# KatherLab/STAMP

Hardware: AMD Instinct MI355X
Metric: tiles/sec encoded (224x224, ViT-L/14) (higher is better)
Workload: dtype f16

## Files before the change

stamp_amd/csrc/gemm_4w16.h:

```cpp
#pragma once
#include <type_traits>
#include "gemm_kernel.h"

namespace amds {

__device__ __forceinline__ f32x4 agpr_read(const f32x4& a) {
    f32x4 v;
    asm("v_accvgpr_read_b32 %0, %1" : "=v"(v[0]) : "a"(a[0]));
    asm("v_accvgpr_read_b32 %0, %1" : "=v"(v[1]) : "a"(a[1]));
    asm("v_accvgpr_read_b32 %0, %1" : "=v"(v[2]) : "a"(a[2]));
    asm("v_accvgpr_read_b32 %0, %1" : "=v"(v[3]) : "a"(a[3]));
    return v;
}

template <typename T, int EPI, int P3 = 6, int P0 = 6, bool SPREAD = true, int PRL = 0, int PRS = 0, bool TN = false>
__global__ void __launch_bounds__(256) __attribute__((amdgpu_waves_per_eu(1, 1)))
gemm_4w16_kernel(const T* __restrict__ A, long lda, const T* __restrict__ W, long ldw, int M, int N, int K,
                 EpiArgs ep, int tiles_m, int tiles_n) {
    typedef typename Act<T>::vec8 vec8;
    typedef typename Act<T>::vec4 vec4;
    constexpr int BM = 256, BN = 256, BK = 64, NT = 256;
    constexpr int ROWB = BK * 2;
    constexpr int A_BYTES = BM * ROWB, STAGE = (BM + BN) * ROWB;
    constexpr int FI = 8, FJ = 8;
    constexpr int GROUP_M = 8;

    extern __shared__ __attribute__((aligned(16))) char smem[];

    const int tid = threadIdx.x;
    const int lane = tid & 63;
    const int wave = __builtin_amdgcn_readfirstlane(tid >> 6);
    const int wm = wave >> 1, wn = wave & 1;
    const int l15 = lane & 15, kb = lane >> 4;
    const int l31 = lane & 31, hi = lane >> 5;

    int tm, tn;
    {
        const int nwg = gridDim.x, bid = blockIdx.x;
        const int xcd = bid & 7, q = nwg >> 3, r = nwg & 7;
        const int t = (xcd < r ? xcd * (q + 1) : r * (q + 1) + (xcd - r) * q) + (bid >> 3);
        const int group = GROUP_M * tiles_n;
        const int g = t / group, first_m = g * GROUP_M;
        const int gm = min(tiles_m - first_m, GROUP_M);
        const int rr = t - g * group;
        tm = first_m + rr % gm;
        tn = rr / gm;
    }
    const int m0 = tm * BM, n0 = tn * BN;
    if (ep.nbatch > 1) {
        const long by = blockIdx.y;
        A += by * ep.bsA;
        W += by * ep.bsW;
        constexpr bool F32O = (EPI == AMDS_EPI_RESIDUAL || EPI == AMDS_EPI_BIAS_F32 || EPI == AMDS_EPI_BIAS_GELU_F32 || EPI == AMDS_EPI_BIAS_RELU_F32);
        if (F32O) ep.out = reinterpret_cast<float*>(ep.out) + by * ep.bsOut;
        else ep.out = reinterpret_cast<T*>(ep.out) + by * ep.bsOut;
    }

    const int rows_a = min(BM, M - m0);
    const long tn_valid = TN ? (ep.ktot > 0 ? min((long)K, ep.ktot - (long)blockIdx.y * K) : (long)K) : 0;
    const __amdgpu_buffer_rsrc_t rsrc_a = TN ? __builtin_amdgcn_make_buffer_rsrc(const_cast<T*>(A + m0), 0, tn_valid > 0 ? (int)(((tn_valid - 1) * lda + BM) * 2) : 0, 0x00020000)
                                             : __builtin_amdgcn_make_buffer_rsrc(const_cast<T*>(A + (long)m0 * lda), 0, (int)((((long)rows_a - 1) * lda + K) * 2), 0x00020000);
    const __amdgpu_buffer_rsrc_t rsrc_w = TN ? __builtin_amdgcn_make_buffer_rsrc(const_cast<T*>(W + n0), 0, tn_valid > 0 ? (int)(((tn_valid - 1) * ldw + BN) * 2) : 0, 0x00020000)
                                             : __builtin_amdgcn_make_buffer_rsrc(const_cast<T*>(W + (long)n0 * ldw), 0, (int)(((long)(BN - 1) * ldw + K) * 2), 0x00020000);
    int voff[16];
#pragma unroll
    for (int it = 0; it < 16; ++it) {
        if constexpr (TN) {
            const int c = (it & 7) * NT + tid, row = c >> 5, pos = c & 31, g = (row & 3) | ((row >> 1) & 4);
            voff[it] = (int)(((long)row * (it < 8 ? lda : ldw) + (pos ^ (g << 1)) * 8) * 2);
        } else {
            const int c = (it & 7) * NT + tid, row = c >> 3, cp = c & 7, sc = cp ^ ((row >> 1) & 7);
            voff[it] = (int)(((long)row * (it < 8 ? lda : ldw) + sc * 8) * 2);
        }
    }
    auto issue_pieces = [&](int kt, int lo, int hi_) {
        char* st = smem + (kt & 1) * STAGE;
        const int koff = TN ? kt * BK * (int)lda * 2 : kt * BK * 2;
        const int koff_w = TN ? kt * BK * (int)ldw * 2 : koff;
#pragma unroll
        for (int it = 0; it < 16; ++it)
            if (it >= lo && it < hi_) {
                if (it < 8) {
                    __builtin_amdgcn_raw_ptr_buffer_load_lds(rsrc_a, (lptr_t)(st + ((it & 7) * NT + wave * 64) * 16), 16, voff[it], koff, 0, 0);
                } else {
                    __builtin_amdgcn_raw_ptr_buffer_load_lds(rsrc_w, (lptr_t)(st + A_BYTES + ((it & 7) * NT + wave * 64) * 16), 16, voff[it], koff_w,
                                                             0, 0);
                }
            }
    };

    const int swz = (l15 >> 1) & 7;
    const int a_off = (wm * 128 + l15) * ROWB;
    const int w_off = A_BYTES + (wn * 128 + l15) * ROWB;

    const bool lnf = ep.rowstat != nullptr;
    const bool bias_in_acc = ep.bias != nullptr && ep.acc_scale == 1.0f && !lnf;
    f32x4 acc[FI][FJ];
    {
        f32x4 b0[FJ];
#pragma unroll
        for (int j = 0; j < FJ; ++j) b0[j] = f32x4{0.f, 0.f, 0.f, 0.f};
        if (bias_in_acc) {
#pragma unroll
            for (int j = 0; j < FJ; ++j) b0[j] = *reinterpret_cast<const f32x4*>(ep.bias + n0 + wn * 128 + j * 16 + 4 * kb);
        }
        __builtin_amdgcn_sched_barrier(0);
        issue_pieces(0, 0, 16);
        if constexpr (P3 < 0) {
            if (K / BK > 1) issue_pieces(1, 0, 16);
        }
        __builtin_amdgcn_sched_barrier(0);
#pragma unroll
        for (int i = 0; i < FI; ++i)
#pragma unroll
            for (int j = 0; j < FJ; ++j) acc[i][j] = b0[j];
    }
#pragma unroll
    for (int i = 0; i < FI; ++i) {
        if (i == FI - 1)
            asm volatile("s_nop 7" : "+a"(acc[i][0]), "+a"(acc[i][1]), "+a"(acc[i][2]), "+a"(acc[i][3]), "+a"(acc[i][4]), "+a"(acc[i][5]),
                         "+a"(acc[i][6]), "+a"(acc[i][7]));
        else
            asm volatile("" : "+a"(acc[i][0]), "+a"(acc[i][1]), "+a"(acc[i][2]), "+a"(acc[i][3]), "+a"(acc[i][4]), "+a"(acc[i][5]),
                         "+a"(acc[i][6]), "+a"(acc[i][7]));
    }
    __builtin_amdgcn_sched_barrier(0);

    vec8 af[2][FI], wf[2][FJ];
    const int tn_g = (l15 >> 2) | ((kb & 1) << 2);
    const int tn_row = (kb * 8 + (l15 >> 2)) * 512 + (l15 & 1) * 8 + ((l15 >> 1) & 1) * 16;
    auto load_frags = [&](int kt, int ks, int s, int lo, int hi_) {
        const char* sb = smem + (kt & 1) * STAGE;
        if constexpr (TN) {
            const unsigned base = (unsigned)(size_t)(sb + tn_row + ks * 32 * 512);
#pragma unroll
            for (int q = 0; q < 16; ++q)
                if (q >= lo && q < hi_) {
                    const int qq = q & 7;
                    const unsigned pq = base + (q < 8 ? 0 : A_BYTES) + ((q < 8 ? wm : wn) * 16 + 2 * (qq ^ tn_g)) * 16;
                    u32x2 a0, a1;
                    asm volatile("ds_read_b64_tr_b16 %0, %1" : "=v"(a0) : "v"(pq) : "memory");
                    asm volatile("ds_read_b64_tr_b16 %0, %1 offset:2048" : "=v"(a1) : "v"(pq) : "memory");
                    const vec8 f = __builtin_bit_cast(vec8, u32x4{a0[0], a0[1], a1[0], a1[1]});
                    if (q < 8) af[s][qq] = f; else wf[s][qq] = f;
                }
        } else {
            const int co = ((ks * 4 + kb) ^ swz) << 4;
#pragma unroll
            for (int q = 0; q < 16; ++q)
                if (q >= lo && q < hi_) {
                    if (q < 8) af[s][q] = *reinterpret_cast<const vec8*>(sb + a_off + q * 16 * ROWB + co);
                    else wf[s][q - 8] = *reinterpret_cast<const vec8*>(sb + w_off + (q - 8) * 16 * ROWB + co);
                }
        }
    };
    auto unit = [&](int s, int ih, auto nr_c, int rkt, int rks, int rs, int rlo, auto nc_c, int ckt, int clo) {
        constexpr int NR = decltype(nr_c)::value, NC = decltype(nc_c)::value;
        constexpr int R_SPAN = SPREAD ? (NR >= 16 ? 16 : 32) : (NR > 0 ? NR : 1), C_LO = SPREAD ? (NR >= 16 ? 16 : 0) : NR,
                      C_SPAN = SPREAD ? 32 - C_LO : (NC > 0 ? NC : 1);
#pragma unroll
        for (int m = 0; m < 32; ++m) {
            Act<T>::mfma16_agpr(wf[s][m & 7], af[s][ih * 4 + (m >> 3)], acc[ih * 4 + (m >> 3)][m & 7]);
            if (NR > 0 && m < R_SPAN) {
                const int r0 = m * NR / R_SPAN, r1 = (m + 1) * NR / R_SPAN;
                if (r1 > r0) load_frags(rkt, rks, rs, rlo + r0, rlo + r1);
            }
            if (NC > 0 && m >= C_LO && m < C_LO + C_SPAN) {
                const int c0 = (m - C_LO) * NC / C_SPAN, c1 = (m - C_LO + 1) * NC / C_SPAN;
// ... 199 lines not shown
                    *reinterpret_cast<vec4*>(smem + row * 256 + ((chunk ^ (row & 15)) << 4) + half) = Act<T>::from_f32x4(o);
                }
        }
        __syncthreads();
        const int l15r = lane & 15, rsub = lane >> 4;
#pragma unroll 4
        for (int it = 0; it < 16; ++it) {
            const int row = wave * 64 + it * 4 + rsub;
            const u32x4 v = *reinterpret_cast<const u32x4*>(smem + row * 256 + l15r * 16);
            const int chunk = l15r ^ (row & 15);
            if (m0 + row < M)
                *reinterpret_cast<u32x4*>(reinterpret_cast<T*>(ep.out) + (long)(m0 + row) * ep.ldo + n0 / 2 + chunk * 8) = v;
        }
        return;
    }
    if constexpr (EPI == AMDS_EPI_RESIDUAL) {
        if (rmw_fast) {
            const int rows_o = min(BM, M - m0);
            rsrc_o = __builtin_amdgcn_make_buffer_rsrc(reinterpret_cast<float*>(ep.out) + (long)m0 * ep.ldo + n0, 0,
                                                       (int)((((long)rows_o - 1) * ep.ldo + BN) * 4), 0x00020000);
#pragma unroll
            for (int h = 0; h < 2; ++h)
#pragma unroll
                for (int u = 0; u < 8; ++u)
                    offu[h][u] = (wave * 64 + 2 * u + hi) * ldo4 + (((l31 >> 4) ^ h) << 9) + (((l31 & 15) ^ (2 * u + hi)) << 4);
            const __amdgpu_buffer_rsrc_t rsrc_h = __builtin_amdgcn_make_buffer_rsrc(
                ep.xh ? reinterpret_cast<T*>(ep.xh) + (long)m0 * ep.ldo + n0 : reinterpret_cast<T*>(ep.out), 0,
                ep.xh ? (int)((((long)rows_o - 1) * ep.ldo + BN) * 2) : 0, 0x00020000);
            const __amdgpu_buffer_rsrc_t rsrc_l = __builtin_amdgcn_make_buffer_rsrc(
                ep.xl ? reinterpret_cast<T*>(ep.xl) + (long)m0 * ep.ldo + n0 : reinterpret_cast<T*>(ep.out), 0,
                ep.xl ? (int)((((long)rows_o - 1) * ep.ldo + BN) * 2) : 0, 0x00020000);
            const int np_part = N / 128;
            auto run = [&](auto has_scale_c, auto lnp_c, auto pl_c) {
                constexpr bool HS = decltype(has_scale_c)::value, LNP = decltype(lnp_c)::value, PL = decltype(pl_c)::value;
                auto load_prev = [&](int pass, int b8) {
                    if constexpr (PL) {
                        int rowoff = b8 * 16 * ldo4 + pass * 256;
                        asm volatile("" : "+s"(rowoff));
#pragma unroll
                        for (int u = 0; u < 8; ++u) {
                            const int o = (offu[b8 & 1][u] + rowoff) >> 1;
                            const u32x2 ph = __builtin_bit_cast(u32x2, __builtin_amdgcn_raw_buffer_load_b64(rsrc_h, o, 0, 0));
                            const u32x2 pl = __builtin_bit_cast(u32x2, __builtin_amdgcn_raw_buffer_load_b64(rsrc_l, o, 0, 0));
                            old[b8][u] = __builtin_bit_cast(f32x4, u32x4{ph[0], ph[1], pl[0], pl[1]});
                        }
                    } else {
                        load_old(pass, b8);
                    }
                };
                f32x4 sc[4];
                auto load_scale = [&](int pass) {
                    if constexpr (HS) {
#pragma unroll
                        for (int jj = 0; jj < 4; ++jj)
                            sc[jj] = *reinterpret_cast<const f32x4*>(ep.scale + n0 + wn * 128 + (pass * 4 + jj) * 16 + 4 * kb);
                    }
                };
                load_scale(0);
#pragma unroll
                for (int b8 = 0; b8 < 4; ++b8) load_prev(0, b8);
#pragma unroll
                for (int pass = 0; pass < 2; ++pass) {
#pragma unroll
                    for (int i = 0; i < FI; ++i) {
                        const int row = wm * 128 + i * 16 + l15;
#pragma unroll
                        for (int jj = 0; jj < 4; ++jj) {
                            f32x4 v = agpr_read(acc[i][pass * 4 + jj]);
                            if constexpr (HS) v *= sc[jj];
                            const int chunk = wn * 16 + jj * 4 + kb;
                            *reinterpret_cast<f32x4*>(smem + row * 512 + ((chunk ^ (row & 31)) << 4)) = v;
                        }
                        __builtin_amdgcn_sched_barrier(0);
                    }
                    asm volatile("s_waitcnt lgkmcnt(0)" ::: "memory");
                    __builtin_amdgcn_sched_barrier(0);
                    __builtin_amdgcn_s_barrier();
                    __builtin_amdgcn_sched_barrier(0);
                    if (pass == 0) load_scale(1);
#pragma unroll
                    for (int b8 = 0; b8 < 4; ++b8) {
                        f32x4 v[8];
#pragma unroll
                        for (int u = 0; u < 8; ++u) {
                            const int row = wave * 64 + (b8 * 8 + u) * 2 + hi;
                            v[u] = *reinterpret_cast<const f32x4*>(smem + row * 512 + l31 * 16);
                        }
                        int rowoff = b8 * 16 * ldo4 + pass * 256;
                        asm volatile("" : "+s"(rowoff));
#pragma unroll
                        for (int u = 0; u < 8; ++u) {
                            if constexpr (PL) {
                                const u32x4 o = __builtin_bit_cast(u32x4, old[b8][u]);
                                const vec4 h4 = __builtin_bit_cast(vec4, u32x2{o[0], o[1]}), l4 = __builtin_bit_cast(vec4, u32x2{o[2], o[3]});
                                f32x4 old4;
                                if constexpr (std::is_same<T, f16>::value) {
                                    old4 = f32x4{mix_add_hh<0, 0>(o[0], o[2]), mix_add_hh<1, 1>(o[0], o[2]), mix_add_hh<0, 0>(o[1], o[3]), mix_add_hh<1, 1>(o[1], o[3])};
                                } else {
                                    old4 = __builtin_convertvector(h4, f32x4) + __builtin_convertvector(l4, f32x4);
                                }
                                v[u] += old4;
                            } else {
                                v[u] += old[b8][u];
                                __builtin_amdgcn_raw_buffer_store_b128(__builtin_bit_cast(u32x4, v[u]), rsrc_o, offu[b8 & 1][u] + rowoff, 0, 0);
                            }
                        }
                        if constexpr (LNP) {
                            f32x2 ss[8];
#pragma unroll
                            for (int u = 0; u < 8; ++u) {
                                const vec4 c = Act<T>::from_f32x4(v[u]);
                                __builtin_amdgcn_raw_buffer_store_b64(__builtin_bit_cast(u32x2, c), rsrc_h, (offu[b8 & 1][u] + rowoff) >> 1, 0, 0);
                                if constexpr (PL) {
                                    f32x4 rest;
                                    if constexpr (std::is_same<T, f16>::value) {
                                        const u32x2 cu = __builtin_bit_cast(u32x2, c);
                                        rest = f32x4{mix_sub_fh<0>(v[u][0], cu[0]), mix_sub_fh<1>(v[u][1], cu[0]), mix_sub_fh<0>(v[u][2], cu[1]), mix_sub_fh<1>(v[u][3], cu[1])};
                                    } else {
                                        rest = v[u] - __builtin_convertvector(c, f32x4);
                                    }
                                    const vec4 cl = Act<T>::from_f32x4(rest);
                                    __builtin_amdgcn_raw_buffer_store_b64(__builtin_bit_cast(u32x2, cl), rsrc_l, (offu[b8 & 1][u] + rowoff) >> 1, 0, 0);
                                }
                                ss[u] = f32x2{(v[u][0] + v[u][1]) + (v[u][2] + v[u][3]),
                                              fmaf(v[u][0], v[u][0], v[u][1] * v[u][1]) + fmaf(v[u][2], v[u][2], v[u][3] * v[u][3])};
                            }
                            const f32x2 tot = half_wave_sum8(ss, l31);
                            const int urow = ((l31 >> 4) & 1) * 4 + ((l31 >> 3) & 1) * 2 + ((l31 >> 2) & 1);
                            const int prow = m0 + wave * 64 + b8 * 16 + 2 * urow + hi;
                            if ((l31 & 3) == 0 && prow < M)
                                *reinterpret_cast<f32x2*>(ep.rowpart + ((long)prow * np_part + tn * 2 + pass) * 2) = tot;
                        }
                        if (pass == 0) load_prev(1, b8);
                        __builtin_amdgcn_sched_barrier(0);
                    }
                    if (pass == 0) {
                        asm volatile("s_waitcnt lgkmcnt(0)" ::: "memory");
                        __builtin_amdgcn_sched_barrier(0);
                        __builtin_amdgcn_s_barrier();
                        __builtin_amdgcn_sched_barrier(0);
                    }
                }
            };
            if (ep.xl) {
                if (ep.scale) run(std::true_type{}, std::true_type{}, std::true_type{}); else run(std::false_type{}, std::true_type{}, std::true_type{});
            } else if (ep.xh) {
                if (ep.scale) run(std::true_type{}, std::true_type{}, std::false_type{}); else run(std::false_type{}, std::true_type{}, std::false_type{});
            } else {
                if (ep.scale) run(std::true_type{}, std::false_type{}, std::false_type{}); else run(std::false_type{}, std::false_type{}, std::false_type{});
            }
            return;
        }
    }
    constexpr int NPASS = F16OUT ? 1 : 2;
    constexpr int JP = FJ / NPASS;
#pragma unroll
    for (int pass = 0; pass < NPASS; ++pass) {
        if (pass) __syncthreads();
        EpiArgs epv = ep;
        if (bias_in_acc || lnf) epv.bias = nullptr;
        EpiCols<JP> cols;
        epi_cols_load<EPI>(epv, cols, [&](int jj) { return n0 + wn * 128 + (pass * JP + jj) * 16 + 4 * kb; });
        auto values = [&](auto fast_c) {
            constexpr bool FAST = decltype(fast_c)::value;
#pragma unroll
            for (int i = 0; i < FI; ++i) {
                const int row = wm * 128 + i * 16 + l15;
#pragma unroll
                for (int jj = 0; jj < JP; jj += 2) {
                    const int j = pass * JP + jj;
                    f32x4 v0 = agpr_read(acc[i][j]), v1 = agpr_read(acc[i][j + 1]);
                    epi_value_pair<EPI, FAST, true>(epv, cols.bias[jj], cols.scale[jj], cols.bias[jj + 1], cols.scale[jj + 1], v0, v1);
                    if constexpr (F16OUT) {
                        const vec4 o0 = Act<T>::from_f32x4(v0), o1 = Act<T>::from_f32x4(v1);
                        const int chunk = wn * 16 + j * 2 + (kb >> 1);
                        const int half = ((kb & 1) ^ ((l15 >> 3) & 1)) * 8;
                        *reinterpret_cast<vec4*>(smem + row * 512 + ((chunk ^ (row & 31)) << 4) + half) = o0;
                        *reinterpret_cast<vec4*>(smem + row * 512 + (((chunk + 2) ^ (row & 31)) << 4) + half) = o1;
                    } else {
                        const int chunk = wn * 16 + jj * 4 + kb;
                        *reinterpret_cast<f32x4*>(smem + row * 512 + ((chunk ^ (row & 31)) << 4)) = v0;
                        *reinterpret_cast<f32x4*>(smem + row * 512 + (((chunk + 4) ^ (row & 31)) << 4)) = v1;
                    }
                }
            }
        };
        auto values_ln = [&]() {
            if constexpr (LNC && F16OUT) {
#pragma unroll
                for (int i = 0; i < FI; ++i) {
                    const int row = wm * 128 + i * 16 + l15;
#pragma unroll
                    for (int j = 0; j < FJ; j += 2) {
                        f32x4 v0 = agpr_read(acc[i][j]), v1 = agpr_read(acc[i][j + 1]);
                        v0 = v0 * rs[i][0] + (cs[j] * rs[i][1] + cb[j]);
                        v1 = v1 * rs[i][0] + (cs[j + 1] * rs[i][1] + cb[j + 1]);
                        epi_value_pair<EPI, true, true>(epv, cb[j], cb[j], cb[j + 1], cb[j + 1], v0, v1);
                        const vec4 o0 = Act<T>::from_f32x4(v0), o1 = Act<T>::from_f32x4(v1);
                        const int chunk = wn * 16 + j * 2 + (kb >> 1);
                        const int half = ((kb & 1) ^ ((l15 >> 3) & 1)) * 8;
                        *reinterpret_cast<vec4*>(smem + row * 512 + ((chunk ^ (row & 31)) << 4) + half) = o0;
                        *reinterpret_cast<vec4*>(smem + row * 512 + (((chunk + 2) ^ (row & 31)) << 4) + half) = o1;
                    }
                }
            }
        };
        if (LNC && F16OUT && lnf) values_ln();
        else if (F16OUT && (bias_in_acc || (ep.bias == nullptr && ep.acc_scale == 1.0f))) values(std::true_type{}); else values(std::false_type{});
        __syncthreads();
#pragma unroll 1
        for (int b8 = 0; b8 < 4; ++b8) {
            if constexpr (F16OUT) {
                u32x4 v[8];
#pragma unroll
                for (int u = 0; u < 8; ++u) {
                    const int row = wave * 64 + (b8 * 8 + u) * 2 + hi;
                    v[u] = *reinterpret_cast<const u32x4*>(smem + row * 512 + l31 * 16);
                    if ((u >> 2) & 1) v[u] = u32x4{v[u][2], v[u][3], v[u][0], v[u][1]};
                }
#pragma unroll
                for (int u = 0; u < 8; ++u) {
                    const int row = wave * 64 + (b8 * 8 + u) * 2 + hi;
                    const int chunk = l31 ^ (row & 31);
                    if (m0 + row < M)
                        *reinterpret_cast<u32x4*>(reinterpret_cast<T*>(ep.out) + (long)(m0 + row) * ep.ldo + n0 + chunk * 8) = v[u];
                }
            } else {
                f32x4 v[8], o[8];
#pragma unroll
                for (int u = 0; u < 8; ++u) {
                    const int row = wave * 64 + (b8 * 8 + u) * 2 + hi;
                    const int chunk = l31 ^ (row & 31);
                    const int n = n0 + (chunk >> 4) * 128 + pass * 64 + (chunk & 15) * 4;
                    v[u] = *reinterpret_cast<const f32x4*>(smem + row * 512 + l31 * 16);
                    if constexpr (EPI == AMDS_EPI_RESIDUAL)
                        o[u] = *reinterpret_cast<const f32x4*>(reinterpret_cast<const float*>(ep.out) +
                                                               (long)min(m0 + row, M - 1) * ep.ldo + n);
                }
#pragma unroll
                for (int u = 0; u < 8; ++u) {
                    const int row = wave * 64 + (b8 * 8 + u) * 2 + hi;
                    const int chunk = l31 ^ (row & 31);
                    const int n = n0 + (chunk >> 4) * 128 + pass * 64 + (chunk & 15) * 4;
                    if constexpr (EPI == AMDS_EPI_RESIDUAL) v[u] += o[u];
                    if (m0 + row < M)
                        *reinterpret_cast<f32x4*>(reinterpret_cast<float*>(ep.out) + (long)(m0 + row) * ep.ldo + n) = v[u];
                }
            }
        }
    }
}

template <typename T, int EPI, bool SPREAD = true, int P3 = 6, int P0 = 6, int PRL = 0, int PRS = 0, bool TN = false>
static int launch_gemm_4w16(const void* A, long lda, const void* W, long ldw, int M, int N, int K, const EpiArgs& ep,
                            hipStream_t st) {
    if constexpr (!epi_is_staged<EPI>() && EPI != AMDS_EPI_SWIGLU) {
        return launch_gemm_4w64<T, EPI>(A, lda, W, ldw, M, N, K, ep, st);
    } else {
        constexpr int LDS = 2 * (256 + 256) * 128;
        constexpr auto kern = gemm_4w16_kernel<T, EPI, P3, P0, SPREAD, PRL, PRS, TN>;
        EpiArgs epp = ep;
        if constexpr (PRL + PRS > 0) {
            static char* scratch = nullptr;
            static size_t scratch_bytes = 0;
            const size_t need = (size_t)cdiv(M, 256) * (N / 256) * (K / 64) * 4096 * (PRL > PRS ? PRL : PRS);
            if (need > scratch_bytes) {
                if (scratch) AMDS_HIP(hipFree(scratch));
                AMDS_HIP(hipMalloc(reinterpret_cast<void**>(&scratch), need));
                scratch_bytes = need;
            }
            epp.pos = reinterpret_cast<const float*>(scratch);
        }
        AMDS_HIP(lds_opt_in<kern>(LDS));
        const int tiles_m = cdiv(M, 256), tiles_n = N / 256;
        hipLaunchKernelGGL(kern, dim3(tiles_m * tiles_n, ep.nbatch), dim3(256), LDS, st, reinterpret_cast<const T*>(A), lda,
                           reinterpret_cast<const T*>(W), ldw, M, N, K, epp, tiles_m, tiles_n);
        AMDS_LAUNCH_CHECK("gemm_4w16_kernel");
        return AMDS_OK;
    }
}

}
```

stamp_amd/csrc/gemm_kernel.h:

```cpp
#pragma once
#include <type_traits>
#include "launch.h"

namespace amds {

struct EpiArgs {
    void* out;
    long ldo;
    const float* bias;
    const float* scale;
    const float* pos;
    int np, T, P;
    float acc_scale;
    long bsA = 0, bsW = 0, bsOut = 0;
    int nbatch = 1;
    void* xh = nullptr;
    void* xl = nullptr;
    float* rowpart = nullptr;
    const float* rowstat = nullptr;
    const float* colsum = nullptr;
    long ktot = 0;
};

template <int EPI>
constexpr bool epi_is_staged() {
    return EPI == AMDS_EPI_BIAS || EPI == AMDS_EPI_BIAS_GELU || EPI == AMDS_EPI_BIAS_RELU || EPI == AMDS_EPI_RESIDUAL ||
           EPI == AMDS_EPI_BIAS_F32 || EPI == AMDS_EPI_BIAS_GELU_F32 || EPI == AMDS_EPI_BIAS_RELU_F32;
}

template <int G>
struct EpiCols {
    f32x4 bias[G], scale[G];
};
template <int EPI, int G, typename F>
__device__ __forceinline__ void epi_cols_load(const EpiArgs& ep, EpiCols<G>& c, F col_of) {
    if (ep.bias) {
#pragma unroll
        for (int q = 0; q < G; ++q) c.bias[q] = *reinterpret_cast<const f32x4*>(ep.bias + col_of(q));
    }
    if constexpr (EPI == AMDS_EPI_RESIDUAL) {
        if (ep.scale) {
#pragma unroll
            for (int q = 0; q < G; ++q) c.scale[q] = *reinterpret_cast<const f32x4*>(ep.scale + col_of(q));
        }
    }
}

template <int EPI>
__device__ __forceinline__ f32x4 epi_value(const EpiArgs& ep, const f32x4& bias, const f32x4& scale, f32x4 v) {
    if (ep.acc_scale != 1.0f) v *= ep.acc_scale;
    if (ep.bias) v += bias;
    if constexpr (EPI == AMDS_EPI_BIAS_GELU) {
        const f32x2 a = gelu_erf_poly2(f32x2{v[0], v[1]}), b = gelu_erf_poly2(f32x2{v[2], v[3]});
        v = f32x4{a[0], a[1], b[0], b[1]};
    }
    if constexpr (EPI == AMDS_EPI_BIAS_GELU_F32) {
#pragma unroll
        for (int e = 0; e < 4; ++e) v[e] = gelu_erf(v[e]);
    }
    if constexpr (EPI == AMDS_EPI_BIAS_RELU || EPI == AMDS_EPI_BIAS_RELU_F32) {
#pragma unroll
        for (int e = 0; e < 4; ++e) v[e] = fmaxf(v[e], 0.f);
    }
    if constexpr (EPI == AMDS_EPI_RESIDUAL) {
        if (ep.scale) v *= scale;
    }
    return v;
}

template <int EPI, bool FAST, bool NOBIAS = false>
__device__ __forceinline__ void epi_value_pair(const EpiArgs& ep, const f32x4& b0, const f32x4& s0, const f32x4& b1, const f32x4& s1,
                                               f32x4& v0, f32x4& v1) {
    if constexpr (FAST && EPI == AMDS_EPI_BIAS_GELU) {
        if constexpr (!NOBIAS) {
            v0 += b0;
            v1 += b1;
        }
        f32x2 q[4] = {f32x2{v0[0], v0[1]}, f32x2{v0[2], v0[3]}, f32x2{v1[0], v1[1]}, f32x2{v1[2], v1[3]}};
        gelu_erf_poly2_n<4>(q);
        v0 = f32x4{q[0][0], q[0][1], q[1][0], q[1][1]};
        v1 = f32x4{q[2][0], q[2][1], q[3][0], q[3][1]};
    } else if constexpr (FAST && (EPI == AMDS_EPI_BIAS || EPI == AMDS_EPI_BIAS_RELU)) {
        if constexpr (!NOBIAS) {
            v0 += b0;
            v1 += b1;
        }
        if constexpr (EPI == AMDS_EPI_BIAS_RELU) {
#pragma unroll
            for (int e = 0; e < 4; ++e) { v0[e] = fmaxf(v0[e], 0.f); v1[e] = fmaxf(v1[e], 0.f); }
        }
    } else {
        v0 = epi_value<EPI>(ep, b0, s0, v0);
        v1 = epi_value<EPI>(ep, b1, s1, v1);
    }
}

template <int EPI, typename T>
__device__ __forceinline__ void epilogue4(const EpiArgs& ep, int m, int n, float v0, float v1, float v2,
                                          float v3) {
    typedef typename Act<T>::vec4 vec4;
    if (ep.acc_scale != 1.0f) { v0 *= ep.acc_scale; v1 *= ep.acc_scale; v2 *= ep.acc_scale; v3 *= ep.acc_scale; }
    if constexpr (EPI != AMDS_EPI_SWIGLU) {
        if (ep.bias) {
            const f32x4 b = *reinterpret_cast<const f32x4*>(ep.bias + n);
            v0 += b[0]; v1 += b[1]; v2 += b[2]; v3 += b[3];
        }
    }
    if constexpr (EPI == AMDS_EPI_BIAS_GELU) {
        v0 = gelu_erf_fast(v0); v1 = gelu_erf_fast(v1); v2 = gelu_erf_fast(v2); v3 = gelu_erf_fast(v3);
    }
    if constexpr (EPI == AMDS_EPI_BIAS_GELU_F32) {
        v0 = gelu_erf(v0); v1 = gelu_erf(v1); v2 = gelu_erf(v2); v3 = gelu_erf(v3);
    }
    if constexpr (EPI == AMDS_EPI_BIAS_RELU || EPI == AMDS_EPI_BIAS_RELU_F32) {
        v0 = fmaxf(v0, 0.f); v1 = fmaxf(v1, 0.f); v2 = fmaxf(v2, 0.f); v3 = fmaxf(v3, 0.f);
    }
    if constexpr (EPI == AMDS_EPI_BIAS || EPI == AMDS_EPI_BIAS_GELU || EPI == AMDS_EPI_BIAS_RELU) {
        vec4 o;
        o[0] = Act<T>::from_f32(v0); o[1] = Act<T>::from_f32(v1);
        o[2] = Act<T>::from_f32(v2); o[3] = Act<T>::from_f32(v3);
        *reinterpret_cast<vec4*>(reinterpret_cast<T*>(ep.out) + (long)m * ep.ldo + n) = o;
    } else if constexpr (EPI == AMDS_EPI_BIAS_F32 || EPI == AMDS_EPI_BIAS_GELU_F32 ||
                         EPI == AMDS_EPI_BIAS_RELU_F32) {
        f32x4 o = {v0, v1, v2, v3};
        *reinterpret_cast<f32x4*>(reinterpret_cast<float*>(ep.out) + (long)m * ep.ldo + n) = o;
    } else if constexpr (EPI == AMDS_EPI_RESIDUAL) {
        if (ep.scale) {
            const f32x4 s = *reinterpret_cast<const f32x4*>(ep.scale + n);
            v0 *= s[0]; v1 *= s[1]; v2 *= s[2]; v3 *= s[3];
        }
        f32x4* p = reinterpret_cast<f32x4*>(reinterpret_cast<float*>(ep.out) + (long)m * ep.ldo + n);
        f32x4 x = *p;
        x[0] += v0; x[1] += v1; x[2] += v2; x[3] += v3;
        *p = x;
    } else if constexpr (EPI == AMDS_EPI_PATCH) {
        const int b = m / ep.np, pi = m - b * ep.np;
        const f32x4 pe = *reinterpret_cast<const f32x4*>(ep.pos + (long)pi * ep.ldo + n);
        f32x4 o = {v0 + pe[0], v1 + pe[1], v2 + pe[2], v3 + pe[3]};
        *reinterpret_cast<f32x4*>(reinterpret_cast<float*>(ep.out) +
                                  ((long)b * ep.T + ep.P + pi) * ep.ldo + n) = o;
    }
}

template <typename T, int BM, int BN, int WM, int WN, int EPI>
__global__ void __launch_bounds__(64 * WM * WN) __attribute__((amdgpu_waves_per_eu(2, 2)))
gemm_tn_kernel(const T* __restrict__ A, long lda, const T* __restrict__ W, long ldw, int M, int N, int K,
               EpiArgs ep, int tiles_m, int tiles_n) {
    typedef typename Act<T>::vec8 vec8;
    typedef typename Act<T>::vec4 vec4;
    constexpr int NT = 64 * WM * WN;
    constexpr int BK = 64;
    constexpr int WTM = BM / WM, WTN = BN / WN;
    constexpr int FM = WTM / 32, FN = WTN / 32;
// ... 59 lines not shown
    const int w_row_off = A_BYTES + (wn * WTN + l31) * 128;

    f32x16 acc[FM][FN];
#pragma unroll
    for (int i = 0; i < FM; ++i)
#pragma unroll
        for (int j = 0; j < FN; ++j)
#pragma unroll
            for (int r = 0; r < 16; ++r) acc[i][j][r] = 0.f;

    const int nk = K / BK;
    stage_load(0, 0);
    vec8 af[2][FM], wf[2][FN];
    auto load_frags = [&](const char* sb, int ks, int set) {
        const int coff = ((ks * 2 + hi) ^ swz) << 4;
#pragma unroll
        for (int i = 0; i < FM; ++i)
            af[set][i] = *reinterpret_cast<const vec8*>(sb + a_row_off + i * 32 * 128 + coff);
#pragma unroll
        for (int j = 0; j < FN; ++j)
            wf[set][j] = *reinterpret_cast<const vec8*>(sb + w_row_off + j * 32 * 128 + coff);
    };
    for (int kt = 0; kt < nk; ++kt) {
        asm volatile("s_waitcnt vmcnt(0)" ::: "memory");
        __syncthreads();
        if (kt + 1 < nk) stage_load((kt + 1) & 1, kt + 1);
        const char* sb = smem + (kt & 1) * STAGE;
        load_frags(sb, 0, 0);
#pragma unroll
        for (int ks = 0; ks < 4; ++ks) {
            if (ks + 1 < 4) load_frags(sb, ks + 1, (ks + 1) & 1);
#pragma unroll
            for (int i = 0; i < FM; ++i)
#pragma unroll
                for (int j = 0; j < FN; ++j)
                    acc[i][j] = Act<T>::mfma32(wf[ks & 1][j], af[ks & 1][i], acc[i][j]);
            if (ks + 1 < 4) {
#pragma unroll
                for (int r = 0; r < PAIRS; ++r) {
                    __builtin_amdgcn_sched_group_barrier(0x008, 1, 0);
                    __builtin_amdgcn_sched_group_barrier(0x100, 1, 0);
                }
                if constexpr (FM * FN > PAIRS) __builtin_amdgcn_sched_group_barrier(0x008, FM * FN - PAIRS, 0);
                if constexpr (FM + FN > PAIRS) __builtin_amdgcn_sched_group_barrier(0x100, FM + FN - PAIRS, 0);
            }
        }
    }

    if constexpr (epi_is_staged<EPI>()) {
        constexpr bool F16OUT = (EPI == AMDS_EPI_BIAS || EPI == AMDS_EPI_BIAS_GELU || EPI == AMDS_EPI_BIAS_RELU);
        constexpr int CPR = BN * (F16OUT ? 2 : 4) / 16, PITCH = (CPR | 1) * 16;
        EpiCols<FN * 4> cols;
        epi_cols_load<EPI>(ep, cols, [&](int q) { return n0 + wn * WTN + (q >> 2) * 32 + 8 * (q & 3) + 4 * hi; });
        __syncthreads();
#pragma unroll
        for (int i = 0; i < FM; ++i) {
            const int row = wm * WTM + i * 32 + l31;
#pragma unroll
            for (int j = 0; j < FN; ++j)
#pragma unroll
                for (int g = 0; g < 4; ++g) {
                    const int nl = wn * WTN + j * 32 + 8 * g + 4 * hi;
                    f32x4 v = {acc[i][j][4 * g], acc[i][j][4 * g + 1], acc[i][j][4 * g + 2], acc[i][j][4 * g + 3]};
                    v = epi_value<EPI>(ep, cols.bias[j * 4 + g], cols.scale[j * 4 + g], v);
                    if constexpr (F16OUT) {
                        vec4 o;
#pragma unroll
                        for (int e = 0; e < 4; ++e) o[e] = Act<T>::from_f32(v[e]);
                        *reinterpret_cast<vec4*>(smem + row * PITCH + nl * 2) = o;
                    } else {
                        *reinterpret_cast<f32x4*>(smem + row * PITCH + nl * 4) = v;
                    }
                }
        }
        __syncthreads();
        for (int idx = tid; idx < BM * CPR; idx += NT) {
            const int row = idx / CPR, c = idx - row * CPR;
            if (m0 + row < M) {
                if constexpr (F16OUT) {
                    const u32x4 v = *reinterpret_cast<const u32x4*>(smem + row * PITCH + c * 16);
                    *reinterpret_cast<u32x4*>(reinterpret_cast<T*>(ep.out) + (long)(m0 + row) * ep.ldo + n0 + c * 8) = v;
                } else {
                    f32x4 v = *reinterpret_cast<const f32x4*>(smem + row * PITCH + c * 16);
                    f32x4* p = reinterpret_cast<f32x4*>(reinterpret_cast<float*>(ep.out) + (long)(m0 + row) * ep.ldo + n0 + c * 4);
                    if constexpr (EPI == AMDS_EPI_RESIDUAL) v += *p;
                    *p = v;
                }
            }
        }
    } else {
#pragma unroll
    for (int i = 0; i < FM; ++i) {
        const int m = m0 + wm * WTM + i * 32 + l31;
        if (m < M) {
            if constexpr (EPI == AMDS_EPI_SWIGLU) {
#pragma unroll
                for (int j = 0; j < FN; j += 2) {
                    const int hbase = (n0 + wn * WTN + j * 32) / 2;
#pragma unroll
                    for (int g = 0; g < 4; ++g) {
                        const int hcol = hbase + 8 * g + 4 * hi;
                        float gte[4], val[4];
                        const f32x4 bg = *reinterpret_cast<const f32x4*>(
                            ep.bias + n0 + wn * WTN + j * 32 + 8 * g + 4 * hi);
                        const f32x4 bv = *reinterpret_cast<const f32x4*>(
                            ep.bias + n0 + wn * WTN + (j + 1) * 32 + 8 * g + 4 * hi);
                        vec4 o;
#pragma unroll
                        for (int e = 0; e < 4; ++e) {
                            gte[e] = acc[i][j][4 * g + e] * ep.acc_scale + bg[e];
                            val[e] = acc[i][j + 1][4 * g + e] * ep.acc_scale + bv[e];
                            o[e] = Act<T>::from_f32(silu(gte[e]) * val[e]);
                        }
                        *reinterpret_cast<vec4*>(reinterpret_cast<T*>(ep.out) + (long)m * ep.ldo + hcol) = o;
                    }
                }
            } else {
#pragma unroll
                for (int j = 0; j < FN; ++j)
#pragma unroll
                    for (int g = 0; g < 4; ++g) {
                        const int n = n0 + wn * WTN + j * 32 + 8 * g + 4 * hi;
                        epilogue4<EPI, T>(ep, m, n, acc[i][j][4 * g + 0], acc[i][j][4 * g + 1],
                                          acc[i][j][4 * g + 2], acc[i][j][4 * g + 3]);
                    }
            }
        }
    }
    }
}

template <typename T, int BM, int BN, int WM, int WN, int EPI>
static int launch_gemm_cfg(const void* A, long lda, const void* W, long ldw, int M, int N, int K,
                           const EpiArgs& ep, hipStream_t st) {
    constexpr int STAGE = (BM + BN) * 64 * 2;
    constexpr int EPI_LDS = BM * ((BN * 4 / 16) | 1) * 16;
    constexpr int LDS = 2 * STAGE > EPI_LDS ? 2 * STAGE : EPI_LDS;
    constexpr auto kern = gemm_tn_kernel<T, BM, BN, WM, WN, EPI>;
    AMDS_HIP(lds_opt_in<kern>(LDS));
    const int tiles_m = cdiv(M, BM), tiles_n = N / BN;
    hipLaunchKernelGGL(kern, dim3(tiles_m * tiles_n), dim3(64 * WM * WN), LDS, st,
                       reinterpret_cast<const T*>(A), lda, reinterpret_cast<const T*>(W), ldw, M, N, K, ep,
                       tiles_m, tiles_n);
    AMDS_LAUNCH_CHECK("gemm_tn_kernel");
    return AMDS_OK;
}

template <typename T, int EPI>
static int launch_gemm_8p64(const void* A, long lda, const void* W, long ldw, int M, int N, int K, const EpiArgs& ep,
                            hipStream_t st);
template <typename T, int EPI>
static int launch_gemm_4w64(const void* A, long lda, const void* W, long ldw, int M, int N, int K, const EpiArgs& ep,
                            hipStream_t st);
template <typename T, int EPI, bool SPREAD, int P3, int P0, int PRL, int PRS, bool TN>
static int launch_gemm_4w16(const void* A, long lda, const void* W, long ldw, int M, int N, int K, const EpiArgs& ep,
                            hipStream_t st);

template <typename T, int EPI>
static int launch_gemm(int cfg, const void* A, long lda, const void* W, long ldw, int M, int N, int K,
                       const EpiArgs& ep, hipStream_t st) {
    if (cfg == 10 && N % 256 == 0 && ep.nbatch == 1) return launch_gemm_4w64<T, EPI>(A, lda, W, ldw, M, N, K, ep, st);
    if (cfg == 10) cfg = 8;
    if (cfg == 12 && N % 256 == 0) return launch_gemm_4w16<T, EPI, true, 6, 6, 0, 0, false>(A, lda, W, ldw, M, N, K, ep, st);
    if (cfg == 13 && N % 256 == 0) return launch_gemm_4w16<T, EPI, true, -2, 0, 0, 0, false>(A, lda, W, ldw, M, N, K, ep, st);
#ifdef AMDS_GEMM_PROBE
    if constexpr (EPI == AMDS_EPI_BIAS || EPI == AMDS_EPI_BIAS_GELU || EPI == AMDS_EPI_RESIDUAL) {
        if (cfg == 21 && N % 256 == 0) return launch_gemm_4w16<T, EPI, true, 6, 6, 0, 2, false>(A, lda, W, ldw, M, N, K, ep, st);
        if (cfg == 22 && N % 256 == 0) return launch_gemm_4w16<T, EPI, true, 6, 6, 1, 1, false>(A, lda, W, ldw, M, N, K, ep, st);
        if (cfg == 23 && N % 256 == 0) return launch_gemm_4w16<T, EPI, true, 6, 6, 4, 4, false>(A, lda, W, ldw, M, N, K, ep, st);
    }
#endif
    if constexpr (EPI == AMDS_EPI_BIAS_F32) {
        if (cfg == 15 && N % 256 == 0 && M % 256 == 0) return launch_gemm_4w16<T, EPI, true, 6, 6, 0, 0, true>(A, lda, W, ldw, M, N, K, ep, st);
    }
    if (cfg == 15) { set_error("amds_gemm: kernel 15 (token-major operands) takes the BIAS_F32 epilogue and M, N multiples of 256"); return AMDS_ERR_INVALID; }
    if (cfg == 12 || cfg == 13) cfg = 8;

    if (cfg == 8 && N % 256 == 0) return launch_gemm_8p64<T, EPI>(A, lda, W, ldw, M, N, K, ep, st);
    if (cfg == 8) cfg = 0;
    if (cfg == 0 && N % 128 != 0) cfg = 1;
    switch (cfg) {
        case 0: return launch_gemm_cfg<T, 128, 128, 2, 2, EPI>(A, lda, W, ldw, M, N, K, ep, st);
        case 1:
            if constexpr (EPI == AMDS_EPI_SWIGLU || EPI == AMDS_EPI_PATCH) {
                set_error("amds_gemm: the 128x96 tile has no SWIGLU / PATCH epilogue");
                return AMDS_ERR_INVALID;
            } else {
                if (N % 96 != 0) { set_error("amds_gemm: kernel 1 needs N %% 96 == 0 (N=%d)", N); return AMDS_ERR_INVALID; }
                return launch_gemm_cfg<T, 128, 96, 4, 1, EPI>(A, lda, W, ldw, M, N, K, ep, st);
            }
    }
    set_error("amds_gemm: unknown tile config %d", cfg);
    return AMDS_ERR_INVALID;
}

template <typename T>
int gemm_dispatch(int cfg, int epi, const void* A, long lda, const void* W, long ldw, int M, int N, int K,
                  const EpiArgs& ep, hipStream_t st);

#define AMDS_GEMM_DISPATCH_IMPL(T)                                                                        \
    template <>                                                                                           \
    int gemm_dispatch<T>(int cfg, int epi, const void* A, long lda, const void* W, long ldw, int M, int N, \
                         int K, const EpiArgs& ep, hipStream_t st) {                                      \
        switch (epi) {                                                                                    \
            case AMDS_EPI_BIAS: return launch_gemm<T, AMDS_EPI_BIAS>(cfg, A, lda, W, ldw, M, N, K, ep, st); \
            case AMDS_EPI_BIAS_GELU: return launch_gemm<T, AMDS_EPI_BIAS_GELU>(cfg, A, lda, W, ldw, M, N, K, ep, st); \
            case AMDS_EPI_BIAS_RELU: return launch_gemm<T, AMDS_EPI_BIAS_RELU>(cfg, A, lda, W, ldw, M, N, K, ep, st); \
            case AMDS_EPI_RESIDUAL: return launch_gemm<T, AMDS_EPI_RESIDUAL>(cfg, A, lda, W, ldw, M, N, K, ep, st); \
            case AMDS_EPI_BIAS_F32: return launch_gemm<T, AMDS_EPI_BIAS_F32>(cfg, A, lda, W, ldw, M, N, K, ep, st); \
            case AMDS_EPI_SWIGLU: return launch_gemm<T, AMDS_EPI_SWIGLU>(cfg, A, lda, W, ldw, M, N, K, ep, st); \
            case AMDS_EPI_PATCH: return launch_gemm<T, AMDS_EPI_PATCH>(cfg, A, lda, W, ldw, M, N, K, ep, st); \
            case AMDS_EPI_BIAS_GELU_F32: return launch_gemm<T, AMDS_EPI_BIAS_GELU_F32>(cfg, A, lda, W, ldw, M, N, K, ep, st); \
            case AMDS_EPI_BIAS_RELU_F32: return launch_gemm<T, AMDS_EPI_BIAS_RELU_F32>(cfg, A, lda, W, ldw, M, N, K, ep, st); \
        }                                                                                                 \
        set_error("amds_gemm: unknown epilogue %d", epi);                                                 \
        return AMDS_ERR_INVALID;                                                                          \
    }

}
```

Baseline: 6041.

## Stream f16 GEMM epilogue through per-wave LDS slabs with buffer stores

Adds a STREAM variant of the 256x256 GEMM epilogue for f16 bias/GELU/ReLU outputs. Each wave converts one 16-row accumulator slice at a time into a double-buffered 8 KB LDS slab, then writes 128-bit rows to global memory with raw buffer stores while the next slice is being converted. This replaces the block-wide staged epilogue and its block barriers with a software-pipelined, wave-local path, so output stores overlap with accumulator conversion. It is on by default for configs 12 and 13, can be disabled through an environment variable, and adds config 14 as the non-streamed fallback.

```diff
diff --git a/stamp_amd/csrc/gemm_4w16.h b/stamp_amd/csrc/gemm_4w16.h
--- a/stamp_amd/csrc/gemm_4w16.h
+++ b/stamp_amd/csrc/gemm_4w16.h
@@ -13,7 +13,7 @@
     return v;
 }
 
-template <typename T, int EPI, int P3 = 6, int P0 = 6, bool SPREAD = true, int PRL = 0, int PRS = 0, bool TN = false>
+template <typename T, int EPI, int P3 = 6, int P0 = 6, bool SPREAD = true, int PRL = 0, int PRS = 0, bool STREAM = false, bool TN = false>
 __global__ void __launch_bounds__(256) __attribute__((amdgpu_waves_per_eu(1, 1)))
 gemm_4w16_kernel(const T* __restrict__ A, long lda, const T* __restrict__ W, long ldw, int M, int N, int K,
                  EpiArgs ep, int tiles_m, int tiles_n) {
@@ -519,6 +519,70 @@
             return;
         }
     }
+    if constexpr (F16OUT && STREAM) {
+        EpiArgs epv = ep;
+        if (bias_in_acc || lnf) epv.bias = nullptr;
+        EpiCols<FJ> cols;
+        epi_cols_load<EPI>(epv, cols, [&](int j) { return n0 + wn * 128 + j * 16 + 4 * kb; });
+        const int rows_o = min(BM, M - m0);
+        const __amdgpu_buffer_rsrc_t rsrc_s = __builtin_amdgcn_make_buffer_rsrc(reinterpret_cast<T*>(ep.out) + (long)m0 * ep.ldo + n0, 0,
+                                                                                (int)((((long)rows_o - 1) * ep.ldo + BN) * 2), 0x00020000);
+        char* slab = smem + wave * 8192;
+        const int wr_base = l15 * 256 + (((kb & 1) ^ (l15 & 1)) << 3);
+        const int wr_x = (kb >> 1) ^ ((l15 >> 1) & 7);
+        const int rd_base = kb * 512 + ((l15 ^ kb) << 4);
+        const int ldo2 = (int)ep.ldo * 2;
+        const int st_base = (wm * 128 + 2 * kb) * ldo2 + (wn * 128 + l15 * 8) * 2;
+        auto run = [&](auto mode_c) {
+            constexpr int MODE = decltype(mode_c)::value;
+            u32x4 rd[4];
+#pragma unroll
+            for (int s = 0; s <= FI; ++s) {
+                if (s < FI) {
+                    char* wp = slab + (s & 1) * 4096 + wr_base;
+#pragma unroll
+                    for (int j = 0; j < FJ; j += 2) {
+                        f32x4 v0 = agpr_read(acc[s][j]), v1 = agpr_read(acc[s][j + 1]);
+                        if constexpr (MODE == 2) {
+                            if constexpr (LNC) {
+                                v0 = v0 * rs[s][0] + (cs[j] * rs[s][1] + cb[j]);
+                                v1 = v1 * rs[s][0] + (cs[j + 1] * rs[s][1] + cb[j + 1]);
+                                epi_value_pair<EPI, true, true>(epv, cb[j], cb[j], cb[j + 1], cb[j + 1], v0, v1);
+                            }
+                        } else {
+                            epi_value_pair<EPI, MODE == 1, true>(epv, cols.bias[j], cols.scale[j], cols.bias[j + 1], cols.scale[j + 1], v0, v1);
+                        }
+                        const vec4 o0 = Act<T>::from_f32x4(v0), o1 = Act<T>::from_f32x4(v1);
+                        *reinterpret_cast<vec4*>(wp + (((2 * j) ^ wr_x) << 4)) = o0;
+                        *reinterpret_cast<vec4*>(wp + (((2 * j + 2) ^ wr_x) << 4)) = o1;
+                    }
+                }
+                __builtin_amdgcn_sched_barrier(0);
+                if (s > 0) {
+#pragma unroll
+                    for (int t = 0; t < 4; ++t) {
+                        const u32x4 v = (t & 1) ? u32x4{rd[t][2], rd[t][3], rd[t][0], rd[t][1]} : rd[t];
+                        const int rowoff = ((s - 1) * 16 + (t & 1) + 8 * (t >> 1)) * ldo2;
+                        __builtin_amdgcn_raw_buffer_store_b128(v, rsrc_s, st_base + rowoff, 0, 0);
+                    }
+                }
+                if (s < FI) {
+                    __builtin_amdgcn_fence(__ATOMIC_ACQ_REL, "wavefront");
+                    __builtin_amdgcn_wave_barrier();
+                    const char* rp = slab + (s & 1) * 4096;
+#pragma unroll
+                    for (int t = 0; t < 4; ++t)
+                        rd[t] = *reinterpret_cast<const u32x4*>(rp + (rd_base ^ ((t >> 1) << 6)) + (t & 1) * 256 + (t >> 1) * 2048);
+                    __builtin_amdgcn_wave_barrier();
+                }
+                __builtin_amdgcn_sched_barrier(0);
+            }
+        };
+        if (LNC && lnf) run(std::integral_constant<int, 2>{});
+        else if (bias_in_acc || (ep.bias == nullptr && ep.acc_scale == 1.0f)) run(std::integral_constant<int, 1>{});
+        else run(std::integral_constant<int, 0>{});
+        return;
+    }
     constexpr int NPASS = F16OUT ? 1 : 2;
     constexpr int JP = FJ / NPASS;
 #pragma unroll
@@ -618,14 +682,18 @@
     }
 }
 
-template <typename T, int EPI, bool SPREAD = true, int P3 = 6, int P0 = 6, int PRL = 0, int PRS = 0, bool TN = false>
+template <typename T, int EPI, bool SPREAD = true, int P3 = 6, int P0 = 6, int PRL = 0, int PRS = 0, bool STREAM = false, bool TN = false>
 static int launch_gemm_4w16(const void* A, long lda, const void* W, long ldw, int M, int N, int K, const EpiArgs& ep,
                             hipStream_t st) {
     if constexpr (!epi_is_staged<EPI>() && EPI != AMDS_EPI_SWIGLU) {
         return launch_gemm_4w64<T, EPI>(A, lda, W, ldw, M, N, K, ep, st);
     } else {
         constexpr int LDS = 2 * (256 + 256) * 128;
-        constexpr auto kern = gemm_4w16_kernel<T, EPI, P3, P0, SPREAD, PRL, PRS, TN>;
+        constexpr bool STR = STREAM && (EPI == AMDS_EPI_BIAS || EPI == AMDS_EPI_BIAS_GELU || EPI == AMDS_EPI_BIAS_RELU);
+        if constexpr (STR) {
+            if (ep.ldo * 512 >= (1L << 31)) return launch_gemm_4w16<T, EPI, SPREAD, P3, P0, PRL, PRS, false, TN>(A, lda, W, ldw, M, N, K, ep, st);
+        }
+        constexpr auto kern = gemm_4w16_kernel<T, EPI, P3, P0, SPREAD, PRL, PRS, STR, TN>;
         EpiArgs epp = ep;
         if constexpr (PRL + PRS > 0) {
             static char* scratch = nullptr;
diff --git a/stamp_amd/csrc/gemm_kernel.h b/stamp_amd/csrc/gemm_kernel.h
--- a/stamp_amd/csrc/gemm_kernel.h
+++ b/stamp_amd/csrc/gemm_kernel.h
@@ -1,4 +1,5 @@
 #pragma once
+#include <stdlib.h>
 #include <type_traits>
 #include "launch.h"
 
@@ -364,29 +365,41 @@
 template <typename T, int EPI>
 static int launch_gemm_4w64(const void* A, long lda, const void* W, long ldw, int M, int N, int K, const EpiArgs& ep,
                             hipStream_t st);
-template <typename T, int EPI, bool SPREAD, int P3, int P0, int PRL, int PRS, bool TN>
+template <typename T, int EPI, bool SPREAD, int P3, int P0, int PRL, int PRS, bool STREAM, bool TN>
 static int launch_gemm_4w16(const void* A, long lda, const void* W, long ldw, int M, int N, int K, const EpiArgs& ep,
                             hipStream_t st);
+
+static inline bool gemm_epi_stream() {
+    const char* e = getenv("AMDS_GEMM_EPI_STREAM");
+    return !(e && *e && atoi(e) == 0);
+}
 
 template <typename T, int EPI>
 static int launch_gemm(int cfg, const void* A, long lda, const void* W, long ldw, int M, int N, int K,
                        const EpiArgs& ep, hipStream_t st) {
     if (cfg == 10 && N % 256 == 0 && ep.nbatch == 1) return launch_gemm_4w64<T, EPI>(A, lda, W, ldw, M, N, K, ep, st);
     if (cfg == 10) cfg = 8;
-    if (cfg == 12 && N % 256 == 0) return launch_gemm_4w16<T, EPI, true, 6, 6, 0, 0, false>(A, lda, W, ldw, M, N, K, ep, st);
-    if (cfg == 13 && N % 256 == 0) return launch_gemm_4w16<T, EPI, true, -2, 0, 0, 0, false>(A, lda, W, ldw, M, N, K, ep, st);
+    if ((cfg == 12 || cfg == 13 || cfg == 14) && N % 256 == 0) {
+        const bool stream = cfg != 14 && gemm_epi_stream();
+        if (cfg == 13) {
+            if (stream) return launch_gemm_4w16<T, EPI, true, -2, 0, 0, 0, true, false>(A, lda, W, ldw, M, N, K, ep, st);
+            return launch_gemm_4w16<T, EPI, true, -2, 0, 0, 0, false, false>(A, lda, W, ldw, M, N, K, ep, st);
+        }
+        if (stream) return launch_gemm_4w16<T, EPI, true, 6, 6, 0, 0, true, false>(A, lda, W, ldw, M, N, K, ep, st);
+        return launch_gemm_4w16<T, EPI, true, 6, 6, 0, 0, false, false>(A, lda, W, ldw, M, N, K, ep, st);
+    }
 #ifdef AMDS_GEMM_PROBE
     if constexpr (EPI == AMDS_EPI_BIAS || EPI == AMDS_EPI_BIAS_GELU || EPI == AMDS_EPI_RESIDUAL) {
-        if (cfg == 21 && N % 256 == 0) return launch_gemm_4w16<T, EPI, true, 6, 6, 0, 2, false>(A, lda, W, ldw, M, N, K, ep, st);
-        if (cfg == 22 && N % 256 == 0) return launch_gemm_4w16<T, EPI, true, 6, 6, 1, 1, false>(A, lda, W, ldw, M, N, K, ep, st);
-        if (cfg == 23 && N % 256 == 0) return launch_gemm_4w16<T, EPI, true, 6, 6, 4, 4, false>(A, lda, W, ldw, M, N, K, ep, st);
+        if (cfg == 21 && N % 256 == 0) return launch_gemm_4w16<T, EPI, true, 6, 6, 0, 2, false, false>(A, lda, W, ldw, M, N, K, ep, st);
+        if (cfg == 22 && N % 256 == 0) return launch_gemm_4w16<T, EPI, true, 6, 6, 1, 1, false, false>(A, lda, W, ldw, M, N, K, ep, st);
+        if (cfg == 23 && N % 256 == 0) return launch_gemm_4w16<T, EPI, true, 6, 6, 4, 4, false, false>(A, lda, W, ldw, M, N, K, ep, st);
     }
 #endif
     if constexpr (EPI == AMDS_EPI_BIAS_F32) {
-        if (cfg == 15 && N % 256 == 0 && M % 256 == 0) return launch_gemm_4w16<T, EPI, true, 6, 6, 0, 0, true>(A, lda, W, ldw, M, N, K, ep, st);
+        if (cfg == 15 && N % 256 == 0 && M % 256 == 0) return launch_gemm_4w16<T, EPI, true, 6, 6, 0, 0, false, true>(A, lda, W, ldw, M, N, K, ep, st);
     }
     if (cfg == 15) { set_error("amds_gemm: kernel 15 (token-major operands) takes the BIAS_F32 epilogue and M, N multiples of 256"); return AMDS_ERR_INVALID; }
-    if (cfg == 12 || cfg == 13) cfg = 8;
+    if (cfg == 12 || cfg == 13 || cfg == 14) cfg = 8;
 
     if (cfg == 8 && N % 256 == 0) return launch_gemm_8p64<T, EPI>(A, lda, W, ldw, M, N, K, ep, st);
     if (cfg == 8) cfg = 0;
```

After: 6203 (median of 6 runs). +2.7%, better.
